# V-DETR/V-DETR

Hardware: AMD Instinct MI355X
Metric: scenes/sec (train fwd+bwd) 40k-pt ScanNet (higher is better)
Workload: dtype f32

## Files before the change

### include/vdetr_hip.h

```cpp
#ifndef VDETR_HIP_H
#define VDETR_HIP_H

#include <stddef.h>
#include <stdint.h>

#ifdef __cplusplus
extern "C" {
#endif

#define VDETR_OK 0
#define VDETR_ERR_ARG 1
#define VDETR_ERR_LAUNCH 2
#define VDETR_ERR_WORKSPACE 3

typedef void* vdetr_stream_t;

int vdetr_abi_version(void);
const char* vdetr_last_error(void);
int vdetr_ab_switches(void);


size_t vdetr_fps_workspace_bytes(int b, int n);
int vdetr_furthest_point_sampling_f32(const float* xyz, int b, int n, int m, int32_t* idx,
                                      void* workspace, size_t workspace_bytes, vdetr_stream_t stream);
// ... 15 lines not shown

int vdetr_ball_query_f32(const float* new_xyz, const float* xyz, int32_t* idx, int b, int n, int m,
                         float radius, int nsample, vdetr_stream_t stream);

int vdetr_group_points_f32(const float* points, const int32_t* idx, float* out, int b, int c, int n,
                           int npoints, int nsample, vdetr_stream_t stream);
int vdetr_group_points_grad_f32(const float* grad_out, const int32_t* idx, float* grad_points, int b,
                                int c, int n, int npoints, int nsample, vdetr_stream_t stream);
int vdetr_group_points_grad_set_f32(const float* grad_out, const int32_t* idx, float* grad_points, int b,
                                    int c, int n, int npoints, int nsample, vdetr_stream_t stream);

int vdetr_three_nn_f32(const float* unknown, const float* known, float* dist2, int32_t* idx, int b,
                       int n, int m, vdetr_stream_t stream);
int vdetr_three_interpolate_f32(const float* points, const int32_t* idx, const float* weight,
                                float* out, int b, int c, int m, int n, vdetr_stream_t stream);
int vdetr_three_interpolate_grad_f32(const float* grad_out, const int32_t* idx, const float* weight,
                                     float* grad_points, int b, int c, int n, int m,
                                     vdetr_stream_t stream);

#define VDETR_ATTN_SHARED_KV 0
#define VDETR_ATTN_PER_HEAD 1

#define VDETR_MASK_NONE 0
#define VDETR_MASK_BOOL 1
#define VDETR_MASK_FLOAT 2

#define VDETR_RPE_BILINEAR 0
#define VDETR_RPE_NEAREST 1

typedef struct vdetr_attn_desc {
  int32_t kind;
  int32_t B, H, nQ, nK;
  float scale;
  const float* table;
  int32_t table_size;
  float log_scale;
  float inv_log_norm;
  int32_t rpe_interp;
  const float* vertices;
  const float* xyz;
  const float* cos_sin;
  const void* mask;
  int32_t mask_kind;
  float dropout_p;
  uint64_t seed, offset;
  const uint64_t* rng_state;
  int32_t k_row_stride, v_row_stride;
  uint32_t* bwd_aux;
  int32_t table_grid;
  int32_t kv_waves;
  int32_t fwd_kernel;
  int32_t bwd_kernel;
  int32_t kv_halves;
  const void* kv_img;
  uint32_t* fwd_sched;
} vdetr_attn_desc;

size_t vdetr_attn_fwd_workspace_bytes(const vdetr_attn_desc* d);
size_t vdetr_attn_kv_image_bytes(int B, int nK);
int vdetr_attn_pack_kv_f32(const float* k, const float* v, int B, int nK, int k_row_stride, int v_row_stride, int nlayers,
                           int64_t layer_stride, void* img, vdetr_stream_t stream);
size_t vdetr_attn_kv_image_parts_bytes(int B, int nK, int parts);
int vdetr_attn_pack_kv_parts_f32(const float* k, const float* v, int B, int nK, int k_row_stride, int v_row_stride, int nlayers,
                                 int64_t layer_stride, int parts, void* img, vdetr_stream_t stream);

int vdetr_attn_fwd_f32(const vdetr_attn_desc* d, const float* q, const float* k, const float* v,
                       float* out, float* lse, float* scores, void* workspace, size_t workspace_bytes,
                       vdetr_stream_t stream);

typedef struct vdetr_attn_parts {
  const float* part_o;
  const float* part_lse;
  int32_t ksplit;
  int32_t reserved;
  int64_t rows;
} vdetr_attn_parts;
int vdetr_attn_fwd_parts_f32(const vdetr_attn_desc* d, const float* q, const float* k, const float* v,
                             float* out, float* lse, float* scores, void* workspace, size_t workspace_bytes,
                             vdetr_attn_parts* parts, vdetr_stream_t stream);

int vdetr_attn_fwd_bf16(const vdetr_attn_desc* d, const void* q, const void* k, const void* v, float* out, float* lse,
                        float* scores, void* workspace, size_t workspace_bytes, vdetr_stream_t stream);
size_t vdetr_attn_bwd_workspace_bytes(const vdetr_attn_desc* d);
int vdetr_attn_bwd_scores_f32(const vdetr_attn_desc* d, const float* scores, const float* dprob, const float* lse,
                              const float* delta, float* probs_out, float* ds_out, float* dtable, void* workspace,
                              size_t workspace_bytes, vdetr_stream_t stream);

size_t vdetr_attn_bwd_kv_workspace_bytes(const vdetr_attn_desc* d);
int vdetr_attn_bwd_kv_f32(const vdetr_attn_desc* d, const float* q, const float* v, const float* dout, const float* scores,
                          const float* lse, const float* delta, float* ds_out, float* dk, float* dv, void* workspace,
                          size_t workspace_bytes, vdetr_stream_t stream);
int vdetr_attn_bwd_kv_delta_f32(const vdetr_attn_desc* d, const float* q, const float* v, const float* dout, const float* out,
                                const float* scores, const float* lse, float* delta, float* ds_out, float* dk, float* dv,
                                void* workspace, size_t workspace_bytes, vdetr_stream_t stream);
typedef struct vdetr_attn_kv_prep {
  int32_t kind, B, H, nQ, nK, v_row_stride;
  const float* q;
  const float* v;
  const float* vertices;
  const float* cos_sin;
  void* workspace;
  float *dk, *dv;
  uint32_t* bwd_aux;
} vdetr_attn_kv_prep;
int vdetr_attn_bwd_kv_prep_f32(const vdetr_attn_kv_prep* items, int n, vdetr_stream_t stream);
int vdetr_attn_bwd_kv_packed_f32(const vdetr_attn_desc* d, const float* q, const float* v, const float* dout, const float* scores,
// ... 989 lines not shown
```

### v-detr_amd/_lib.py

```python
import ctypes
import os

import torch

_HERE = os.path.dirname(os.path.abspath(__file__))
LIB_PATH = os.path.join(_HERE, "lib", "libvdetr_hip.so")

c_int, c_float, c_void_p, c_size_t = ctypes.c_int, ctypes.c_float, ctypes.c_void_p, ctypes.c_size_t

VDETR_ATTN_SHARED_KV, VDETR_ATTN_PER_HEAD = 0, 1
VDETR_MASK_NONE, VDETR_MASK_BOOL, VDETR_MASK_FLOAT = 0, 1, 2
VDETR_RPE_BILINEAR, VDETR_RPE_NEAREST = 0, 1


class AttnDesc(ctypes.Structure):

    _fields_ = [
        ("kind", ctypes.c_int32), ("B", ctypes.c_int32), ("H", ctypes.c_int32), ("nQ", ctypes.c_int32),
        ("nK", ctypes.c_int32), ("scale", c_float),
        ("table", c_void_p), ("table_size", ctypes.c_int32), ("log_scale", c_float), ("inv_log_norm", c_float),
        ("rpe_interp", ctypes.c_int32),
        ("vertices", c_void_p), ("xyz", c_void_p), ("cos_sin", c_void_p),
        ("mask", c_void_p), ("mask_kind", ctypes.c_int32),
        ("dropout_p", c_float), ("seed", ctypes.c_uint64), ("offset", ctypes.c_uint64),
        ("rng_state", c_void_p),
        ("k_row_stride", ctypes.c_int32), ("v_row_stride", ctypes.c_int32),
        ("bwd_aux", c_void_p),
        ("table_grid", ctypes.c_int32), ("kv_waves", ctypes.c_int32), ("fwd_kernel", ctypes.c_int32), ("bwd_kernel", ctypes.c_int32), ("kv_halves", ctypes.c_int32), ("kv_img", c_void_p),
        ("fwd_sched", c_void_p),
    ]


VDETR_CLS_SOFTMAX, VDETR_CLS_SIGMOID = 0, 1

_BOX_IN = ("center", "size", "angle_cls", "angle_res", "cls", "pre_center_norm", "pre_size_norm", "dims_min", "dims_max")
_BOX_OUT = ("center_reg", "size_reg", "center_unnorm", "center_norm", "size_unnorm", "size_norm", "pre_center_unnorm",
            "pre_size_unnorm", "angle_residual", "angle_cont", "angle_prob", "angle_class", "corners", "corners_aa",
            "cls_prob", "objectness")


class BoxDecodeDesc(ctypes.Structure):

    _fields_ = ([(n, ctypes.c_int32) for n in ("B", "N", "A", "C1", "num_angle_bin", "cls_kind")] +
                [(n, c_void_p) for n in _BOX_IN + _BOX_OUT] + [("in_batch_stride", ctypes.c_int32)] +
                [(n, c_void_p) for n in ("cls_logits_t", "angle_logits_t", "angle_res_norm_t", "corners_lidar", "center_size")])


_BOX_GRAD_IN = ("center_reg", "size_reg", "center_unnorm", "center_norm", "size_unnorm", "size_norm", "angle_residual",
                "angle_cont", "angle_prob", "corners", "corners_aa")
_BOX_GRAD_OUT = ("d_center", "d_size", "d_angle_cls", "d_angle_res")


class BoxDecodeGrads(ctypes.Structure):

    _fields_ = ([(n, c_void_p) for n in _BOX_GRAD_IN + _BOX_GRAD_OUT] +
                [(n, c_void_p) for n in ("cls_logits_t", "angle_logits_t", "angle_res_norm_t", "d_cls")] +
                [("out_batch_stride", ctypes.c_int32), ("slab_rows", ctypes.c_int32)])


class AddLnDesc(ctypes.Structure):

    _fields_ = [("rows", ctypes.c_int32), ("C", ctypes.c_int32), ("eps", c_float), ("dropout_p", c_float),
                ("seed", ctypes.c_uint64), ("offset", ctypes.c_uint64), ("rng_state", c_void_p)] + [
        (n, c_void_p) for n in ("x", "r", "gamma", "beta", "gamma2", "beta2", "y", "out", "out2", "mean", "rstd")]


class AddLnGrads(ctypes.Structure):

    _fields_ = [(n, c_void_p) for n in ("d_out", "d_out2", "d_y", "d_x", "d_r", "d_gamma", "d_beta", "d_gamma2", "d_beta2",
                                        "partials")]


class AddLnReduce(ctypes.Structure):

    _fields_ = [("partials", c_void_p), ("nparts", ctypes.c_int32), ("C", ctypes.c_int32), ("d_gamma", c_void_p), ("d_beta", c_void_p),
                ("d_gamma2", c_void_p), ("d_beta2", c_void_p)]


class RbLinear(ctypes.Structure):

    _fields_ = [("w", c_void_p), ("b", c_void_p), ("wt", c_void_p)]
# ... 713 lines not shown
```

### v-detr_amd/attention.py

```python
import contextlib
import ctypes
import os
import weakref

import torch
from torch.autograd import Function

from . import _lib as L

HEAD_DIM = 64


class RPEConfig:

    INTERP = {"bilinear": L.VDETR_RPE_BILINEAR, "nearest": L.VDETR_RPE_NEAREST}

    def __init__(self, table_size=10, log_scale=512.0, max_value=4.0, interp="bilinear"):
        if interp not in self.INTERP:
            raise NotImplementedError(f"RPE interpolation '{interp}' (built: 'bilinear' and 'nearest')")
        self.interp = interp
        self.table_size = int(table_size)
        self.log_scale = float(log_scale)
        self.max_value = float(max_value)

    @property
    def inv_log_norm(self):
        return 1.0 / (3.0 * self.max_value)


def new_rng_state(device, seed=None):
    if seed is None:
        seed = torch.initial_seed()
    return torch.tensor([seed & 0x7FFFFFFFFFFFFFFF, 0], dtype=torch.int64, device=device)


FWD_KERNEL = int(os.environ.get("VDETR_FWD_KERNEL", "0"))
BWD_KERNEL = int(os.environ.get("VDETR_BWD_KERNEL", "0"))
TABLE_GRID = 0
FUSED_KV_BWD = os.environ.get("VDETR_BWD_FUSED", "1") != "0"
SELF_FWD_BODY = os.environ.get("VDETR_SELF_FWD", "") == "body"


_ASYNC_ENV = os.environ.get("VDETR_BWD_ASYNC_TABLE", "auto")
ASYNC_TABLE_GRAD = _ASYNC_ENV != "0"
ASYNC_MIN_PAIRS = 1 << 21
ASYNC_TABLE_GRID = int(os.environ.get("VDETR_BWD_ASYNC_GRID", "190"))


_step_side = {}


def side_branch_in_use(device):
    return bool(_step_side.get(_dev_key(device)))


class SideResults:
    pending = []

    @classmethod
    def flush(cls):
        from .helpers import DeferredParamGrads
        items, cls.pending = cls.pending, []
        late, side_late[:] = list(side_late), []
        for fn, alive in late:
            with torch.no_grad():
                items.append((None, fn(), alive))
        for dev, pairs, _alive in items:
            side = _side_streams.get(_dev_key(dev)) if dev is not None else None
            if side is not None:
                torch.cuda.current_stream(dev).wait_stream(side)
            roots, grads = [], []
            with torch.no_grad():
                for p, g in pairs:
                    if p is not None and p.requires_grad:
                        DeferredParamGrads._deliver(p, g, roots, grads)
            if roots:
                torch.autograd.backward(roots, grads)


_tick = {}
side_late = []


def flush_layer_params_on_side(ref, rows):
    from .helpers import DeferredParamGrads, DeferredPosEmbedGrads
    if not (ref.is_cuda and DeferredParamGrads.enabled and side_branch_in_use(ref.device)):
        return
    dev = ref.device
    key = _dev_key(dev)
    cur = torch.cuda.current_stream(dev)
    fork = torch.cuda.Event()
    fork.record(cur)
    if key not in _tick:
# ... 475 lines not shown
            if 2 <= parts.ksplit <= 16:
                _pending_parts[out.data_ptr()] = (parts, ws, lse, out)
            elif parts.ksplit != 1:
                raise RuntimeError(f"fused_attention: {parts.ksplit} key chunks left unmerged and no consumer takes that many")
        else:
            fwd = lib.vdetr_attn_fwd_bf16 if bf16 else lib.vdetr_attn_fwd_f32
            L.check(fwd(ctypes.byref(d), L.ptr(q), L.ptr(k), L.ptr(v), L.ptr(out), L.ptr(lse),
                        L.ptr(scores), L.ptr(ws), nbytes, L.stream_ptr()), "attn_fwd")
        if need_grad:
            ctx.save_for_backward(q, k, v, table, vertices, xyz, cos_sin, mask, out, lse, scores, rng)
            ctx.cfg = (kind, H, scale, rpe, dropout_p if use_drop else 0.0, salt)
            ctx.kv_rec = None if (bf16 or mask is not None) else _kv_register(out, q, v, table, vertices, cos_sin, kind, B, H, nQ, nK)
            ctx.table_async = bool(table_async)
            ctx.boxes = bool(boxes)
            if table_async and table is not None and table.requires_grad and _async_wanted(q.shape[0], q.shape[1], k.shape[1]):
                _step_side[_dev_key(q.device)] = True
        if _kv_by_out and getattr(ctx, "kv_rec", None) is None:
            _kv_by_out.pop(out.data_ptr(), None)
        return out

    @staticmethod
    def backward(ctx, dout):
        q, k, v, table, vertices, xyz, cos_sin, mask, out, lse, scores, rng = ctx.saved_tensors
        kind, H, scale, rpe, dropout_p, salt = ctx.cfg
        in_dtype = q.dtype
        if in_dtype == torch.bfloat16:
            q, k, v = q.float(), k.float().contiguous(), v.float().contiguous()
        B, nQ, C = q.shape
        nK = k.shape[1]
        lib = L.lib()
        dout = dout.contiguous()
        shared = kind == L.VDETR_ATTN_SHARED_KV
        want_table = table is not None and ctx.needs_input_grad[3]
        d = _desc(kind, B, H, nQ, nK, scale, table, rpe, vertices, xyz, cos_sin, mask, dropout_p, rng, salt, 0, v.stride(1))
        if getattr(ctx, "boxes", False) and BWD_KERNEL == 0 and cos_sin is None:
            d.bwd_kernel = 2
        if want_table:
            aux = _take_zeros(q, (8,), torch.int32)
            d.bwd_aux = aux.data_ptr()
        delta = torch.empty((B, nQ, H) if shared else (B, H, nQ), dtype=torch.float32, device=q.device)
        rows_kv, nprob_kv = (4 * nQ, B) if shared else (nQ, B * H)
        fused = (FUSED_KV_BWD and ((shared and H == 4) or (not shared and not want_table))
                 and rows_kv * nK * 4 < (1 << 31) and nprob_kv <= 65535 and v.stride(1) % 4 == 0
                 and all(t.data_ptr() % 16 == 0 for t in (v, lse)))
        if not fused:
            L.check(lib.vdetr_attn_delta_f32(ctypes.byref(d), L.ptr(dout), L.ptr(out), L.ptr(v), L.ptr(delta), L.stream_ptr()),
                    "attn_delta")
        if fused:
            ds = torch.empty_like(scores)
            dkv = torch.empty((2, B, nK, k.shape[2]), dtype=torch.float32, device=q.device)
            run_async = want_table and ctx.table_async and _async_wanted(B, nQ, nK)
            d.kv_waves = 4 if (run_async or _side_keep) and ASYNC_TABLE_GRID >= 256 else 8
            d.kv_halves = 1 if (_side_keep and not shared) else 2
            rec = getattr(ctx, "kv_rec", None)
            if (rec is not None and rec.prepared and rec.emitted == dout.data_ptr() and (rec.aux is not None) == bool(want_table)
                    and in_dtype == torch.float32):
                delta, dkv, aux = rec.delta, rec.dkv, rec.aux
                d.bwd_aux = aux.data_ptr() if aux is not None else None
                L.check(lib.vdetr_attn_bwd_kv_packed_f32(ctypes.byref(d), L.ptr(q), L.ptr(v), L.ptr(dout), L.ptr(scores), L.ptr(lse),
                                                         L.ptr(delta), L.ptr(ds), L.ptr(dkv[0]), L.ptr(dkv[1]), L.ptr(rec.ws), rec.nbytes,
                                                         L.stream_ptr()), "attn_bwd_kv_packed")
            else:
                nbytes = lib.vdetr_attn_bwd_kv_workspace_bytes(ctypes.byref(d))
                ws = L.workspace(nbytes, q.device)
                L.check(lib.vdetr_attn_bwd_kv_delta_f32(ctypes.byref(d), L.ptr(q), L.ptr(v), L.ptr(dout), L.ptr(out), L.ptr(scores),
                                                        L.ptr(lse), L.ptr(delta), L.ptr(ds), L.ptr(dkv[0]), L.ptr(dkv[1]), L.ptr(ws),
                                                        nbytes, L.stream_ptr()), "attn_bwd_kv")
            from .runtime import ts_mark
            ts_mark("main: key-side pass done" if shared else "main: self-attention key-side pass done")
            dtable = fork = None
            if run_async:
                dtable = _table_accumulator(table)
                fork = torch.cuda.Event()
                fork.record(torch.cuda.current_stream(q.device))
            if shared:
                dq = q.new_empty((B, nQ * H, HEAD_DIM))
                torch.baddbmm(dq, ds.view(B, nQ * H, nK), k, beta=0.0, alpha=float(scale), out=dq)
                dq = dq.view(B, nQ, C)
            else:
                ds_r = ds.view(B * H, nQ, nK)
                k4 = k.reshape(B, nK, H, HEAD_DIM).permute(0, 2, 1, 3)
                if B == 1:
                    dq = q.new_empty((1, nQ, C))
                    dq_r = dq.view(nQ, H, HEAD_DIM).permute(1, 0, 2)
                    torch.baddbmm(dq_r, ds_r, k4[0], beta=0.0, alpha=float(scale), out=dq_r)
                else:
                    dq = torch.bmm(ds_r, k4.reshape(B * H, nK, HEAD_DIM)).mul_(float(scale))
                    dq = dq.view(B, H, nQ, HEAD_DIM).permute(0, 2, 1, 3).reshape(B, nQ, C)
            if want_table:
                if run_async:
                    dtable = _launch_table_async(lib, d, q, ds, table, aux, vertices, xyz, mask, fork, dtable, also=(cos_sin, rng))
                else:
                    dtable = _table_accumulator(table)
                    nbytes = lib.vdetr_attn_bwd_workspace_bytes(ctypes.byref(d))
                    ws = L.workspace(nbytes, q.device)
                    L.check(lib.vdetr_attn_bwd_table_f32(ctypes.byref(d), L.ptr(ds), L.ptr(dtable), L.ptr(ws), nbytes,
                                                         L.stream_ptr()), "attn_bwd_table")
            dk, dv = dkv[0], dkv[1]
            if in_dtype == torch.bfloat16:
                dq, dk, dv = dq.to(in_dtype), dk.to(in_dtype), dv.to(in_dtype)
            return (dq, dk, dv, dtable) + (None,) * 17
        if shared:
            do_r = dout.view(B, nQ * H, HEAD_DIM)
            dprob = torch.bmm(do_r, v.transpose(1, 2))
        else:
            def heads(t, n):
# ... 135 lines not shown
```

### v-detr_amd/csrc/attn_bwd_kv.hip

```cpp
#include "kv_pack.h"
#include "workspace.h"

#include <stdlib.h>

#include <atomic>

namespace vdetr {

int attn_fill_params(const vdetr_attn_desc* d, AttnParams* P, const char* op);

typedef float f32x16 __attribute__((ext_vector_type(16)));


struct KvParams {
  AttnParams A;
  const float* dout;
  float* dk;
  float* dv;
  uint4* pack;
  int R, NT;
};

struct KvProblem {
  const float* q;
  const float* dout;
  const float* v;
  float* dk;
  float* dv;
  size_t score_off;
  size_t row_off;
  int rstride, ostride, b, head;
};
template <bool PERHEAD>
__device__ __forceinline__ KvProblem kv_problem(const KvParams& K, int prob) {
  const AttnParams& P = K.A;
  KvProblem p;
  if (PERHEAD) {
    const int b = prob / P.H, hh = prob - b * P.H, C = P.H * kDh;
    p.b = b; p.head = hh;
    p.q = P.q + (size_t)b * P.nQ * C + hh * kDh;
    p.dout = K.dout + (size_t)b * P.nQ * C + hh * kDh;
    p.rstride = C;
    p.v = P.v + (size_t)b * P.nK * P.v_stride + hh * kDh;
    p.dk = K.dk + (size_t)b * P.nK * C + hh * kDh;
    p.dv = K.dv + (size_t)b * P.nK * C + hh * kDh;
    p.ostride = C;
  } else {
    p.b = prob; p.head = 0;
    p.q = P.q + (size_t)prob * K.R * kDh;
    p.dout = K.dout + (size_t)prob * K.R * kDh;
    p.rstride = kDh;
    p.v = P.v + (size_t)prob * P.nK * P.v_stride;
    p.dk = K.dk + (size_t)prob * P.nK * kDh;
    p.dv = K.dv + (size_t)prob * P.nK * kDh;
    p.ostride = kDh;
  }
  p.score_off = (size_t)prob * K.R * P.nK;
  p.row_off = (size_t)prob * K.R;
  return p;
}


__device__ __forceinline__ f32x16 kv_mfma(bf16x8 a, bf16x8 b, f32x16 c) {
  return __builtin_amdgcn_mfma_f32_32x32x16_bf16(a, b, c, 0, 0, 0);
}
__device__ __forceinline__ f32x16 kv_mfma3(bf16x8 ah, bf16x8 al, bf16x8 bh, bf16x8 bl, f32x16 c) {
  c = kv_mfma(al, bh, c);
  c = kv_mfma(ah, bl, c);
  return kv_mfma(ah, bh, c);
}

template <bool PERHEAD>
__global__ __launch_bounds__(256) void attn_bwd_kv_pack_kernel(KvParams K, DeltaArgs D, int ndelta) {
  if ((int)blockIdx.x < ndelta) {
    __shared__ float wmax[4];
    attn_delta_body(D, (int)blockIdx.x, wmax);
    return;
  }
  const AttnParams& P = K.A;
  const int R = K.R, NT = K.NT;
  const int nprob = PERHEAD ? P.B * P.H : P.B;
  const long gid = (long)((int)blockIdx.x - ndelta) * 256 + threadIdx.x, stride = (long)((int)gridDim.x - ndelta) * 256;
  const long nunits = (long)nprob * NT * 12 * kWave;
  for (long u = gid; u < nunits; u += stride) {
    const int lane = (int)(u & 63);
    long r = u >> 6;
    const int sub = (int)(r & 3);
    r >>= 2;
    const int kind = (int)(r % 3);
    const long bt = r / 3;
    const int prob = (int)(bt / NT), tile = (int)(bt - (long)prob * NT), r0 = tile * 32;
    const int l31 = lane & 31, g = lane >> 5;
    const KvProblem pb = kv_problem<PERHEAD>(K, prob);
    const float* src = kind == 2 ? pb.q : pb.dout;
    float x[8];
    if (kind == 0) {
      const int row = r0 + l31;
#pragma unroll
      for (int e = 0; e < 8; ++e) x[e] = row < R ? src[(size_t)row * pb.rstride + 16 * sub + 8 * g + e] : 0.f;
    } else {
      const int d = 32 * (sub >> 1) + l31, t = sub & 1;
#pragma unroll
      for (int e = 0; e < 8; ++e) {
        const int row = r0 + kv_row(8 * t + e, g);
        x[e] = row < R ? src[(size_t)row * pb.rstride + d] : 0.f;
      }
    }
    bf16x8 hi, lo;
    kv_split8(x, hi, lo);
    uint4* dst = K.pack + ((bt * 3 + kind) * 4 + sub) * kKvOperandUnits;
    dst[lane] = __builtin_bit_cast(uint4, hi);
    dst[kWave + lane] = __builtin_bit_cast(uint4, lo);
  }
  const long nz = (long)P.B * P.nK * (PERHEAD ? P.H : 1) * kDh / 4;
  f32x4* zk = reinterpret_cast<f32x4*>(K.dk);
  f32x4* zv = reinterpret_cast<f32x4*>(K.dv);
  for (long i = gid; i < nz; i += stride) {
    zk[i] = f32x4{0.f, 0.f, 0.f, 0.f};
    zv[i] = f32x4{0.f, 0.f, 0.f, 0.f};
  }
}

template <bool PERHEAD, int WAVES, int HALVES = 2>
// ... 263 lines not shown
    const long bt = u >> 8;
    const int prob = (int)(bt / NT), tile = (int)(bt - (long)prob * NT), r0 = tile * 32;
    const int l31 = ln & 31, g = ln >> 5, d = 32 * (sub >> 1) + l31, t = sub & 1;
    const float* src;
    int rstride;
    if (I.perhead) {
      const int b = prob / I.H, hh = prob - b * I.H;
      src = I.q + (size_t)b * I.nQ * C + hh * kDh;
      rstride = C;
    } else {
      src = I.q + (size_t)prob * R * kDh;
      rstride = kDh;
    }
    float x[8];
#pragma unroll
    for (int e = 0; e < 8; ++e) {
      const int row = r0 + kv_row(8 * t + e, g);
      x[e] = row < R ? src[(size_t)row * rstride + d] : 0.f;
    }
    kv_store_unit(I.pack, bt, 2, sub, ln, x);
  }
  const long nz = (long)I.B * I.nK * (I.perhead ? I.H : 1) * kDh / 4;
  f32x4* zk = reinterpret_cast<f32x4*>(I.dk);
  f32x4* zv = reinterpret_cast<f32x4*>(I.dv);
  for (long i = gid; i < nz; i += stride) {
    zk[i] = f32x4{0.f, 0.f, 0.f, 0.f};
    zv[i] = f32x4{0.f, 0.f, 0.f, 0.f};
  }
}

}

using namespace vdetr;

static bool kv_supported(const vdetr_attn_desc* d) {
  return d && ((d->kind == VDETR_ATTN_SHARED_KV && d->H == 4) || d->kind == VDETR_ATTN_PER_HEAD);
}
static size_t kv_rows(const vdetr_attn_desc* d) { return d->kind == VDETR_ATTN_PER_HEAD ? (size_t)d->nQ : (size_t)d->nQ * 4; }
static size_t kv_problems(const vdetr_attn_desc* d) { return d->kind == VDETR_ATTN_PER_HEAD ? (size_t)d->B * d->H : (size_t)d->B; }

static uint4* lay_out(Carver& c, const vdetr_attn_desc* d) {
  const size_t nt = (kv_rows(d) + 31) / 32;
  return c.take_unpadded<uint4>(kv_problems(d) * nt * kKvTileUnits);
}

extern "C" size_t vdetr_attn_bwd_kv_workspace_bytes(const vdetr_attn_desc* d) {
  if (!kv_supported(d) || d->B <= 0 || d->nQ <= 0 || d->H <= 0) return 0;
  Carver c(nullptr);
  lay_out(c, d);
  return c.bytes() + 256;
}

template <bool PERHEAD, int WAVES, int HALVES = 2>
static int kv_launch(const KvParams& K, int nkt, int nprob, long pack_work, const DeltaArgs& D, int ndelta, bool packed, hipStream_t st) {
  const unsigned pack_blocks = (unsigned)((pack_work + 255) / 256 < 2048 ? (pack_work + 255) / 256 : 2048);
  if (!packed) {
    hipLaunchKernelGGL(attn_bwd_kv_pack_kernel<PERHEAD>, dim3(pack_blocks + (unsigned)ndelta), dim3(256), 0, st, K, D, ndelta);
    if (int e = check_launch("attn_bwd_kv_pack")) return e;
  }
  const size_t strips = (size_t)WAVES * 8 * kWave * sizeof(uint4), tree = (size_t)(WAVES / 2) * 64 * kWave * sizeof(float);
  const size_t fin = (size_t)2 * 32 * (kDh + 1) * sizeof(float);
  const size_t lds = strips > tree ? (strips > fin ? strips : fin) : (tree > fin ? tree : fin);
  if (int e = set_lds(attn_bwd_kv_kernel<PERHEAD, WAVES, HALVES>, lds, "attn_bwd_kv")) return e;
  hipLaunchKernelGGL((attn_bwd_kv_kernel<PERHEAD, WAVES, HALVES>), dim3(HALVES * nkt, nprob), dim3(WAVES * kWave), lds, st, K);
  return check_launch("attn_bwd_kv");
}

static int kv_run(const vdetr_attn_desc* d, const float* q, const float* v, const float* dout, const float* out,
                  const float* scores, const float* lse, float* delta, float* ds_out, float* dk, float* dv, void* workspace,
                  size_t workspace_bytes, vdetr_stream_t stream, bool packed = false) {
  KvParams K;
  if (int e = attn_fill_params(d, &K.A, "attn_bwd_kv")) return e;
  VDETR_REQUIRE(kv_supported(d), "attn_bwd_kv: built for shared K/V with 4 heads and for per-head K/V (kind %d, H %d)", d->kind, d->H);
  VDETR_REQUIRE(q && v && dout && scores && lse && delta && ds_out && dk && dv, "attn_bwd_kv: null pointer");
  VDETR_REQUIRE(K.A.v_stride % 4 == 0 && (((uintptr_t)v | (uintptr_t)lse | (uintptr_t)delta | (uintptr_t)dk | (uintptr_t)dv) & 15) == 0,
                "attn_bwd_kv: v rows, lse, delta, dk and dv must be 16-B aligned");
  const size_t rows = kv_rows(d), nprob = kv_problems(d);
  VDETR_REQUIRE(rows * d->nK * 4 < ((size_t)1 << 31), "attn_bwd_kv: a score matrix (%zu x %d) must stay below 2 GB", rows, d->nK);
  VDETR_REQUIRE(nprob <= 65535, "attn_bwd_kv: %zu score matrices > 65535", nprob);
  if (int e = require_workspace("attn_bwd_kv", workspace, workspace_bytes, vdetr_attn_bwd_kv_workspace_bytes(d))) return e;
  K.A.q = q; K.A.v = v;
  K.A.scores = const_cast<float*>(scores); K.A.lse = const_cast<float*>(lse); K.A.delta = delta; K.A.ds_out = ds_out;
  K.dout = dout; K.dk = dk; K.dv = dv;
  Carver carver(workspace);
  K.pack = lay_out(carver, d);
  K.R = (int)rows;
  K.NT = (K.R + 31) / 32;
  const long units = (long)nprob * K.NT * 12 * kWave;
  const long zero4 = (long)d->B * d->nK * (d->kind == VDETR_ATTN_PER_HEAD ? d->H : 1) * kDh / 4;
  const long work = units > zero4 ? units : zero4;
  const int nkt = (d->nK + 31) / 32;
  VDETR_REQUIRE(d->kv_waves == 0 || d->kv_waves == 4 || d->kv_waves == 8, "attn_bwd_kv: kv_waves %d (0, 4 or 8)", d->kv_waves);
  VDETR_REQUIRE(d->kv_halves == 0 || d->kv_halves == 1 || d->kv_halves == 2, "attn_bwd_kv: kv_halves %d (0, 1 or 2)", d->kv_halves);
  const bool four = d->kv_waves == 4;
  const bool one = d->kv_halves == 1 && !four;
  hipStream_t st = (hipStream_t)stream;
  DeltaArgs D{};
  int ndelta = 0;
  if (out) {
    VDETR_REQUIRE(!d->bwd_aux || d->kind == VDETR_ATTN_SHARED_KV, "attn_bwd_kv: bwd_aux needs the shared-KV kind");
    attn_delta_args(d, dout, out, v, delta, &D);
    ndelta = D.qblocks + D.vblocks;
  }
  if (d->kind == VDETR_ATTN_PER_HEAD) {
    if (one) return kv_launch<true, 8, 1>(K, nkt, (int)nprob, work, D, ndelta, packed, st);
    return four ? kv_launch<true, 4>(K, nkt, (int)nprob, work, D, ndelta, packed, st) : kv_launch<true, 8>(K, nkt, (int)nprob, work, D, ndelta, packed, st);
  }
  if (one) return kv_launch<false, 8, 1>(K, nkt, (int)nprob, work, D, ndelta, packed, st);
  return four ? kv_launch<false, 4>(K, nkt, (int)nprob, work, D, ndelta, packed, st) : kv_launch<false, 8>(K, nkt, (int)nprob, work, D, ndelta, packed, st);
}

extern "C" int vdetr_attn_bwd_kv_f32(const vdetr_attn_desc* d, const float* q, const float* v, const float* dout,
                                     const float* scores, const float* lse, const float* delta, float* ds_out, float* dk,
                                     float* dv, void* workspace, size_t workspace_bytes, vdetr_stream_t stream) {
  return kv_run(d, q, v, dout, nullptr, scores, lse, const_cast<float*>(delta), ds_out, dk, dv, workspace, workspace_bytes, stream);
}

extern "C" int vdetr_attn_bwd_kv_delta_f32(const vdetr_attn_desc* d, const float* q, const float* v, const float* dout,
                                           const float* out, const float* scores, const float* lse, float* delta, float* ds_out,
                                           float* dk, float* dv, void* workspace, size_t workspace_bytes, vdetr_stream_t stream) {
  VDETR_REQUIRE(out, "attn_bwd_kv_delta: null pointer (out)");
  return kv_run(d, q, v, dout, out, scores, lse, delta, ds_out, dk, dv, workspace, workspace_bytes, stream);
}

extern "C" int vdetr_attn_bwd_kv_packed_f32(const vdetr_attn_desc* d, const float* q, const float* v, const float* dout, const float* scores,
                                            const float* lse, const float* delta, float* ds_out, float* dk, float* dv, void* workspace,
                                            size_t workspace_bytes, vdetr_stream_t stream) {
  VDETR_REQUIRE(workspace && (((uintptr_t)workspace) & 255) == 0, "attn_bwd_kv_packed: the workspace (the operand images) must be 256-B aligned");
  return kv_run(d, q, v, dout, nullptr, scores, lse, const_cast<float*>(delta), ds_out, dk, dv, workspace, workspace_bytes, stream, true);
}

extern "C" int vdetr_attn_bwd_kv_prep_f32(const vdetr_attn_kv_prep* items, int n, vdetr_stream_t stream) {
  VDETR_REQUIRE(items && n >= 1 && n <= kPrepMax, "attn_bwd_kv_prep: %d items (1..%d)", n, kPrepMax);
  PrepBatch Bt;
  long blocks = 1;
  for (int i = 0; i < n; ++i) {
    const vdetr_attn_kv_prep& s = items[i];
    VDETR_REQUIRE(s.q && s.v && s.workspace && s.dk && s.dv, "attn_bwd_kv_prep: null pointer in item %d", i);
    VDETR_REQUIRE(s.kind == VDETR_ATTN_SHARED_KV || s.kind == VDETR_ATTN_PER_HEAD, "attn_bwd_kv_prep: kind %d", s.kind);
    VDETR_REQUIRE(s.B > 0 && s.nQ > 0 && s.nK > 0 && s.H == 4, "attn_bwd_kv_prep: item %d: B=%d nQ=%d nK=%d H=%d (4 heads)", i, s.B, s.nQ, s.nK, s.H);
    VDETR_REQUIRE((((uintptr_t)s.workspace) & 255) == 0 && (((uintptr_t)s.dk | (uintptr_t)s.dv) & 15) == 0, "attn_bwd_kv_prep: item %d: alignment", i);
    VDETR_REQUIRE(s.kind == VDETR_ATTN_SHARED_KV || !s.bwd_aux, "attn_bwd_kv_prep: bwd_aux needs the shared-KV kind");
    PrepItem& I = Bt.it[i];
    I.q = s.q; I.v = s.v; I.vertices = s.vertices; I.cos_sin = s.vertices ? s.cos_sin : nullptr;
    I.pack = reinterpret_cast<uint4*>(s.workspace); I.dk = s.dk; I.dv = s.dv; I.aux = s.bwd_aux;
    I.B = s.B; I.H = s.H; I.nQ = s.nQ; I.nK = s.nK;
    I.perhead = s.kind == VDETR_ATTN_PER_HEAD ? 1 : 0;
    I.v_stride = s.v_row_stride ? s.v_row_stride : (I.perhead ? s.H * 64 : 64);
    const long nvb = s.bwd_aux ? ((long)s.B * s.nK + 4 * kDeltaKeys - 1) / (4 * kDeltaKeys) : 0;
    const long nqb = (s.bwd_aux && s.vertices) ? ((long)s.B * s.nQ + 3) / 4 : 0;
    const long R = I.perhead ? s.nQ : (long)s.H * s.nQ, NT = (R + 31) / 32, nprob = I.perhead ? (long)s.B * s.H : s.B;
    const long units = nprob * NT * 4 * kWave, zero4 = (long)s.B * s.nK * (I.perhead ? s.H : 1) * kDh / 4;
    long work = ((units > zero4 ? units : zero4) + 255) / 256;
    work = work < 1 ? 1 : (work > 512 ? 512 : work);
    blocks = blocks > nvb + nqb + work ? blocks : nvb + nqb + work;
  }
  for (int i = n; i < kPrepMax; ++i) Bt.it[i] = Bt.it[0];
// ... 4 lines not shown
```

### v-detr_amd/csrc/kv_pack.h

```cpp
#pragma once
#include "attn_common.h"

namespace vdetr {

typedef __bf16 bf16x8 __attribute__((ext_vector_type(8)));

constexpr int kKvOperandUnits = 2 * kWave;
constexpr int kKvTileUnits = 3 * 4 * kKvOperandUnits;

__device__ __forceinline__ constexpr int kv_row(int v, int g) { return (v & 3) + 8 * (v >> 2) + 4 * g; }

__device__ __forceinline__ void kv_split8(const float (&x)[8], bf16x8& hi, bf16x8& lo) {
#pragma unroll
  for (int e = 0; e < 8; ++e) {
    const __bf16 h = (__bf16)x[e];
    hi[e] = h;
    lo[e] = (__bf16)(x[e] - (float)h);
  }
}

__device__ __forceinline__ void kv_store_unit(uint4* pack, long tile, int kind, int sub, int lane, const float (&x)[8]) {
  bf16x8 hi, lo;
  kv_split8(x, hi, lo);
  uint4* dst = pack + ((tile * 3 + kind) * 4 + sub) * kKvOperandUnits;
  dst[lane] = __builtin_bit_cast(uint4, hi);
  dst[kWave + lane] = __builtin_bit_cast(uint4, lo);
}

struct KvEmit {
  uint4* pack;
  float* delta;
  const float* out;
  unsigned* aux;
  int per_head, nQ;
};
__device__ __forceinline__ void kv_emit_rows16(const KvEmit& E, const float* xs, int stride, int q0, int tid, float* wmax) {
  const int NT = E.per_head ? E.nQ / 32 : E.nQ / 8;
  {
    const int pair = tid >> 2, quarter = tid & 3, ql = pair >> 2, h = pair & 3;
    const float* orow = E.out + ((size_t)(q0 + ql) * 4 + h) * kDh + 16 * quarter;
    const float* drow = xs + ql * stride + h * kDh + 16 * quarter;
    float s = 0.f, n2 = 0.f;
#pragma unroll
    for (int i = 0; i < 4; ++i) {
      const f32x4 o = *reinterpret_cast<const f32x4*>(orow + 4 * i);
      const f32x4 g = *reinterpret_cast<const f32x4*>(drow + 4 * i);
#pragma unroll
      for (int e = 0; e < 4; ++e) { s = fmaf(g[e], o[e], s); n2 = fmaf(g[e], g[e], n2); }
    }
    s += dpp_f32<kDppQuadXor1>(s); s += dpp_f32<kDppQuadXor2>(s);
    n2 += dpp_f32<kDppQuadXor1>(n2); n2 += dpp_f32<kDppQuadXor2>(n2);
    if (quarter == 0) E.delta[E.per_head ? (size_t)h * E.nQ + q0 + ql : (size_t)(q0 + ql) * 4 + h] = s;
    if (E.aux) {
      for (int m = 32; m >= 1; m >>= 1) n2 = fmaxf(n2, __shfl_xor(n2, m, 64));
      if ((tid & 63) == 0) wmax[tid >> 6] = n2;
    }
  }
#pragma unroll
  for (int u = 0; u < 4; ++u) {
    const int id = tid + 256 * u;
    float x[8];
    if (!E.per_head) {
      const int tl = id >> 9, unit = (id >> 6) & 7, lane = id & 63, kind = unit >> 2, sub = unit & 3, l31 = lane & 31, g = lane >> 5;
      if (kind == 0) {
        const float* src = xs + (tl * 8 + (l31 >> 2)) * stride + (l31 & 3) * kDh + 16 * sub + 8 * g;
        const f32x4 a = *reinterpret_cast<const f32x4*>(src), b = *reinterpret_cast<const f32x4*>(src + 4);
#pragma unroll
        for (int e = 0; e < 4; ++e) { x[e] = a[e]; x[4 + e] = b[e]; }
      } else {
        const int d = 32 * (sub >> 1) + l31, t = sub & 1;
#pragma unroll
        for (int e = 0; e < 8; ++e) {
          const int row = kv_row(8 * t + e, g);
          x[e] = xs[(tl * 8 + (row >> 2)) * stride + (row & 3) * kDh + d];
        }
      }
      kv_store_unit(E.pack, (long)(q0 >> 3) + tl, kind, sub, lane, x);
    } else {
      const int head = id >> 8, rem = id & 255, half = (q0 >> 4) & 1;
// ... 24 lines not shown
```

Before: 164.1.

## Add lean per-head self-attention backward dK/dV kernel with split-K slot reduction

Adds a dedicated per-head backward kernel that computes dV and dK for two 32-key tiles per block. Eight waves split the query tiles across slots, using software-pipelined buffer loads and split-bf16 MFMA, then combine partial accumulators with an LDS tree reduction. It is selected automatically when the per-head problem is unmasked, 32-aligned and uses eight waves, replacing the existing kv_launch path. The aim is better occupancy and less per-problem overhead in self-attention backward, at the cost of a new reduction path and extra LDS traffic.

After: 163.0. About the same (-0.6%).

```diff
diff --git a/include/vdetr_hip.h b/include/vdetr_hip.h
--- a/include/vdetr_hip.h
+++ b/include/vdetr_hip.h
@@ -91,6 +91,7 @@
   int32_t fwd_kernel;
   int32_t bwd_kernel;
   int32_t kv_halves;
+  int32_t kv_kernel;
   const void* kv_img;
   uint32_t* fwd_sched;
 } vdetr_attn_desc;
diff --git a/v-detr_amd/_lib.py b/v-detr_amd/_lib.py
--- a/v-detr_amd/_lib.py
+++ b/v-detr_amd/_lib.py
@@ -26,7 +26,7 @@
         ("rng_state", c_void_p),
         ("k_row_stride", ctypes.c_int32), ("v_row_stride", ctypes.c_int32),
         ("bwd_aux", c_void_p),
-        ("table_grid", ctypes.c_int32), ("kv_waves", ctypes.c_int32), ("fwd_kernel", ctypes.c_int32), ("bwd_kernel", ctypes.c_int32), ("kv_halves", ctypes.c_int32), ("kv_img", c_void_p),
+        ("table_grid", ctypes.c_int32), ("kv_waves", ctypes.c_int32), ("fwd_kernel", ctypes.c_int32), ("bwd_kernel", ctypes.c_int32), ("kv_halves", ctypes.c_int32), ("kv_kernel", ctypes.c_int32), ("kv_img", c_void_p),
         ("fwd_sched", c_void_p),
     ]
 
diff --git a/v-detr_amd/attention.py b/v-detr_amd/attention.py
--- a/v-detr_amd/attention.py
+++ b/v-detr_amd/attention.py
@@ -39,6 +39,7 @@
 TABLE_GRID = 0
 FUSED_KV_BWD = os.environ.get("VDETR_BWD_FUSED", "1") != "0"
 SELF_FWD_BODY = os.environ.get("VDETR_SELF_FWD", "") == "body"
+SELF_BWD_BODY = False
 
 
 _ASYNC_ENV = os.environ.get("VDETR_BWD_ASYNC_TABLE", "auto")
@@ -620,6 +621,7 @@
             run_async = want_table and ctx.table_async and _async_wanted(B, nQ, nK)
             d.kv_waves = 4 if (run_async or _side_keep) and ASYNC_TABLE_GRID >= 256 else 8
             d.kv_halves = 1 if (_side_keep and not shared) else 2
+            d.kv_kernel = 1 if SELF_BWD_BODY else 0
             rec = getattr(ctx, "kv_rec", None)
             if (rec is not None and rec.prepared and rec.emitted == dout.data_ptr() and (rec.aux is not None) == bool(want_table)
                     and in_dtype == torch.float32):
diff --git a/v-detr_amd/csrc/attn_bwd_kv.hip b/v-detr_amd/csrc/attn_bwd_kv.hip
--- a/v-detr_amd/csrc/attn_bwd_kv.hip
+++ b/v-detr_amd/csrc/attn_bwd_kv.hip
@@ -8,67 +8,10 @@
 namespace vdetr {
 
 int attn_fill_params(const vdetr_attn_desc* d, AttnParams* P, const char* op);
-
-typedef float f32x16 __attribute__((ext_vector_type(16)));
-
-
-struct KvParams {
-  AttnParams A;
-  const float* dout;
-  float* dk;
-  float* dv;
-  uint4* pack;
-  int R, NT;
-};
-
-struct KvProblem {
-  const float* q;
-  const float* dout;
-  const float* v;
-  float* dk;
-  float* dv;
-  size_t score_off;
-  size_t row_off;
-  int rstride, ostride, b, head;
-};
-template <bool PERHEAD>
-__device__ __forceinline__ KvProblem kv_problem(const KvParams& K, int prob) {
-  const AttnParams& P = K.A;
-  KvProblem p;
-  if (PERHEAD) {
-    const int b = prob / P.H, hh = prob - b * P.H, C = P.H * kDh;
-    p.b = b; p.head = hh;
-    p.q = P.q + (size_t)b * P.nQ * C + hh * kDh;
-    p.dout = K.dout + (size_t)b * P.nQ * C + hh * kDh;
-    p.rstride = C;
-    p.v = P.v + (size_t)b * P.nK * P.v_stride + hh * kDh;
-    p.dk = K.dk + (size_t)b * P.nK * C + hh * kDh;
-    p.dv = K.dv + (size_t)b * P.nK * C + hh * kDh;
-    p.ostride = C;
-  } else {
-    p.b = prob; p.head = 0;
-    p.q = P.q + (size_t)prob * K.R * kDh;
-    p.dout = K.dout + (size_t)prob * K.R * kDh;
-    p.rstride = kDh;
-    p.v = P.v + (size_t)prob * P.nK * P.v_stride;
-    p.dk = K.dk + (size_t)prob * P.nK * kDh;
-    p.dv = K.dv + (size_t)prob * P.nK * kDh;
-    p.ostride = kDh;
-  }
-  p.score_off = (size_t)prob * K.R * P.nK;
-  p.row_off = (size_t)prob * K.R;
-  return p;
-}
-
-
-__device__ __forceinline__ f32x16 kv_mfma(bf16x8 a, bf16x8 b, f32x16 c) {
-  return __builtin_amdgcn_mfma_f32_32x32x16_bf16(a, b, c, 0, 0, 0);
-}
-__device__ __forceinline__ f32x16 kv_mfma3(bf16x8 ah, bf16x8 al, bf16x8 bh, bf16x8 bl, f32x16 c) {
-  c = kv_mfma(al, bh, c);
-  c = kv_mfma(ah, bl, c);
-  return kv_mfma(ah, bh, c);
-}
+bool attn_bwd_self_eligible(const vdetr_attn_desc* d);
+int attn_bwd_self_launch(const KvParams& K, int nprob, hipStream_t st);
+
+
 
 template <bool PERHEAD>
 __global__ __launch_bounds__(256) void attn_bwd_kv_pack_kernel(KvParams K, DeltaArgs D, int ndelta) {
@@ -438,12 +381,14 @@
 }
 
 template <bool PERHEAD, int WAVES, int HALVES = 2>
-static int kv_launch(const KvParams& K, int nkt, int nprob, long pack_work, const DeltaArgs& D, int ndelta, bool packed, hipStream_t st) {
+static int kv_launch(const KvParams& K, int nkt, int nprob, long pack_work, const DeltaArgs& D, int ndelta, bool packed, hipStream_t st,
+                     bool lean = false) {
   const unsigned pack_blocks = (unsigned)((pack_work + 255) / 256 < 2048 ? (pack_work + 255) / 256 : 2048);
   if (!packed) {
     hipLaunchKernelGGL(attn_bwd_kv_pack_kernel<PERHEAD>, dim3(pack_blocks + (unsigned)ndelta), dim3(256), 0, st, K, D, ndelta);
     if (int e = check_launch("attn_bwd_kv_pack")) return e;
   }
+  if (lean) return attn_bwd_self_launch(K, nprob, st);
   const size_t strips = (size_t)WAVES * 8 * kWave * sizeof(uint4), tree = (size_t)(WAVES / 2) * 64 * kWave * sizeof(float);
   const size_t fin = (size_t)2 * 32 * (kDh + 1) * sizeof(float);
   const size_t lds = strips > tree ? (strips > fin ? strips : fin) : (tree > fin ? tree : fin);
@@ -489,6 +434,7 @@
     ndelta = D.qblocks + D.vblocks;
   }
   if (d->kind == VDETR_ATTN_PER_HEAD) {
+    if (attn_bwd_self_eligible(d)) return kv_launch<true, 8, 1>(K, nkt, (int)nprob, work, D, ndelta, packed, st, true);
     if (one) return kv_launch<true, 8, 1>(K, nkt, (int)nprob, work, D, ndelta, packed, st);
     return four ? kv_launch<true, 4>(K, nkt, (int)nprob, work, D, ndelta, packed, st) : kv_launch<true, 8>(K, nkt, (int)nprob, work, D, ndelta, packed, st);
   }
diff --git a/v-detr_amd/csrc/attn_bwd_self.hip b/v-detr_amd/csrc/attn_bwd_self.hip
--- /dev/null
+++ b/v-detr_amd/csrc/attn_bwd_self.hip
@@ -0,0 +1,248 @@
+#include "kv_pack.h"
+
+namespace vdetr {
+
+constexpr int kSbWaves = 8;
+constexpr int kSbSlots = 4;
+constexpr int kSbStripFloats = 2 * 8 * kWave * 4;
+constexpr int kSbLdsFloats = kSbStripFloats + kSbWaves * 64 * kWave;
+constexpr int kSbFinStride = kDh + 1;
+
+template <bool DROP>
+__global__ __launch_bounds__(kSbWaves * kWave) void attn_bwd_self_kernel(KvParams K) {
+  extern __shared__ __attribute__((aligned(16))) float smem[];
+  float* red = smem + kSbStripFloats;
+  AttnParams P = K.A;
+  if (DROP) attn_load_rng(P);
+  const int tid = threadIdx.x, lane = tid & 63;
+  const int w = __builtin_amdgcn_readfirstlane(tid >> 6);
+  const int j = w & 1, slot = w >> 1;
+  const int l31 = lane & 31, g = lane >> 5;
+  const int prob = blockIdx.y, nK = P.nK, NT = K.NT, nkt = nK >> 5;
+  const int kt = 2 * (int)blockIdx.x + j;
+  const bool live = kt < nkt;
+  const KvProblem pb = kv_problem<true>(K, prob);
+  const int key = kt * 32 + l31;
+
+  uint4* vstrip = reinterpret_cast<uint4*>(smem) + j * (8 * kWave) + lane;
+  if (live && slot == 0) {
+    const float* vrow = pb.v + (size_t)key * P.v_stride + 8 * g;
+#pragma unroll
+    for (int s = 0; s < 4; ++s) {
+      const f32x4 a = *reinterpret_cast<const f32x4*>(vrow + 16 * s), c = *reinterpret_cast<const f32x4*>(vrow + 16 * s + 4);
+      const float x[8] = {a[0], a[1], a[2], a[3], c[0], c[1], c[2], c[3]};
+      bf16x8 hi, lo;
+      kv_split8(x, hi, lo);
+      vstrip[(2 * s) * kWave] = __builtin_bit_cast(uint4, hi);
+      vstrip[(2 * s + 1) * kWave] = __builtin_bit_cast(uint4, lo);
+    }
+  }
+  __syncthreads();
+
+  f32x16 accV[2], accK[2];
+#pragma unroll
+  for (int i = 0; i < 16; ++i) { accV[0][i] = 0.f; accV[1][i] = 0.f; accK[0][i] = 0.f; accK[1][i] = 0.f; }
+
+  auto put = [&](int region) {
+    float* dst = red + (size_t)region * 64 * kWave + lane;
+#pragma unroll
+    for (int i = 0; i < 16; ++i) {
+      dst[i * kWave] = accV[0][i]; dst[(16 + i) * kWave] = accV[1][i];
+      dst[(32 + i) * kWave] = accK[0][i]; dst[(48 + i) * kWave] = accK[1][i];
+    }
+  };
+  auto add = [&](int region) {
+    const float* src = red + (size_t)region * 64 * kWave + lane;
+#pragma unroll
+    for (int i = 0; i < 16; ++i) {
+      accV[0][i] += src[i * kWave]; accV[1][i] += src[(16 + i) * kWave];
+      accK[0][i] += src[(32 + i) * kWave]; accK[1][i] += src[(48 + i) * kWave];
+    }
+  };
+  bool parked = false;
+  if (live && slot < NT) {
+    using rsrc_t = __amdgpu_buffer_rsrc_t;
+    const unsigned recs = (unsigned)((size_t)K.R * nK * 4);
+    const rsrc_t rs = __builtin_amdgcn_make_buffer_rsrc(P.scores + pb.score_off, 0, (int)recs, 0x00020000);
+    const rsrc_t rd = __builtin_amdgcn_make_buffer_rsrc(P.ds_out + pb.score_off, 0, (int)recs, 0x00020000);
+    const rsrc_t rl = __builtin_amdgcn_make_buffer_rsrc(const_cast<float*>(P.lse + pb.row_off), 0, K.R * 4, 0x00020000);
+    const rsrc_t rq = __builtin_amdgcn_make_buffer_rsrc(const_cast<float*>(P.delta + pb.row_off), 0, K.R * 4, 0x00020000);
+    const rsrc_t rp = __builtin_amdgcn_make_buffer_rsrc(K.pack + (size_t)prob * NT * kKvTileUnits, 0, NT * kKvTileUnits * 16, 0x00020000);
+    const int rowbytes = nK * 4;
+    const int lane_off = 4 * g * rowbytes + key * 4;
+    const int lane16 = lane * 16, g16 = g * 16;
+    const bool second = (pb.head & 2) != 0;
+    const int shift = (pb.head & 1) * 16;
+
+    float sv[16];
+    f32x4 lq[4], dq[4];
+    auto unit = [&](int tile, int u) {
+      return __builtin_bit_cast(uint4, __builtin_amdgcn_raw_buffer_load_b128(rp, lane16 + (u & 3) * (kWave * 16), (tile * 6 + (u >> 2)) * (4 * kWave * 16), 0));
+    };
+    auto load_dp = [&](int tile, uint4 (&S)[8]) {
+#pragma unroll
+      for (int i = 0; i < 8; ++i) S[i] = unit(tile, i);
+    };
+    auto load_step = [&](int tile, int t, uint4 (&S)[8]) {
+#pragma unroll
+      for (int mt = 0; mt < 2; ++mt)
+#pragma unroll
+        for (int hl = 0; hl < 2; ++hl) {
+          S[2 * mt + hl] = unit(tile, (4 + 2 * mt + t) * 2 + hl);
+          S[4 + 2 * mt + hl] = unit(tile, (8 + 2 * mt + t) * 2 + hl);
+        }
+    };
+    auto load_rows = [&](int tile, int t) {
+#pragma unroll
+      for (int a2 = 0; a2 < 2; ++a2) {
+        const int a = 2 * t + a2;
+#pragma unroll
+        for (int h = 0; h < 4; ++h)
+          sv[4 * a + h] = __builtin_bit_cast(float, __builtin_amdgcn_raw_buffer_load_b32(rs, lane_off, (tile * 32 + 8 * a + h) * rowbytes, kStreamAux));
+        lq[a] = __builtin_bit_cast(f32x4, __builtin_amdgcn_raw_buffer_load_b128(rl, g16, (tile * 8 + 2 * a) * 16, 0));
+        dq[a] = __builtin_bit_cast(f32x4, __builtin_amdgcn_raw_buffer_load_b128(rq, g16, (tile * 8 + 2 * a) * 16, 0));
+      }
+    };
+
+    auto step = [&](uint4 (&X)[8], uint4 (&Y)[8], int tile, int next) {
+      const int r0 = tile * 32;
+      const bool more = next >= 0;
+      unsigned mine = 0;
+      if (DROP) mine = attn_prefix(P, pb.b, r0 + kv_row(l31 & 15, g), pb.head >> 2);
+      f32x16 dp;
+#pragma unroll
+      for (int i = 0; i < 16; ++i) dp[i] = 0.f;
+#pragma unroll
+      for (int s = 0; s < 4; ++s) {
+        const bf16x8 vh = __builtin_bit_cast(bf16x8, vstrip[(2 * s) * kWave]), vl = __builtin_bit_cast(bf16x8, vstrip[(2 * s + 1) * kWave]);
+        dp = kv_mfma3(__builtin_bit_cast(bf16x8, X[2 * s]), __builtin_bit_cast(bf16x8, X[2 * s + 1]), vh, vl, dp);
+      }
+      __builtin_amdgcn_sched_barrier(0);
+      load_step(tile, 1, X);
+      __builtin_amdgcn_sched_barrier(0);
+#pragma unroll
+      for (int t = 0; t < 2; ++t) {
+        float xp[8], xs[8];
+        unsigned word[8];
+        if (DROP) {
+#pragma unroll
+          for (int e = 0; e < 8; ++e)
+            word[e] = drop_word((unsigned)__builtin_amdgcn_ds_bpermute((32 * g + 8 * t + e) << 2, (int)mine), (unsigned)key);
+          if (second) {
+#pragma unroll
+            for (int e = 0; e < 8; ++e) word[e] = drop_next(word[e]);
+          }
+        }
+#pragma unroll
+        for (int a2 = 0; a2 < 2; ++a2) {
+          const int a = 2 * t + a2;
+#pragma unroll
+          for (int h = 0; h < 4; ++h) {
+            const int v = 4 * a + h, e = 4 * a2 + h;
+            const bool keep = DROP ? ((word[e] >> shift) & 0xFFFFu) >= P.drop_thresh : true;
+            const ScoreGrad gr = score_grad(sv[v], lq[a][h], keep, P.drop_scale, true, dp[v], dq[a][h], false);
+            xp[e] = gr.p_drop;
+            xs[e] = gr.ds;
+            __builtin_amdgcn_raw_buffer_store_b32(__float_as_int(gr.ds), rd, lane_off, (r0 + 8 * a + h) * rowbytes, kStreamAux);
+          }
+        }
+        bf16x8 ph, pl, sh, sl;
+        kv_split8(xp, ph, pl);
+        kv_split8(xs, sh, sl);
+        const uint4* op = t ? X : Y;
+#pragma unroll
+        for (int mt = 0; mt < 2; ++mt) {
+          accV[mt] = kv_mfma3(__builtin_bit_cast(bf16x8, op[2 * mt]), __builtin_bit_cast(bf16x8, op[2 * mt + 1]), ph, pl, accV[mt]);
+          accK[mt] = kv_mfma3(__builtin_bit_cast(bf16x8, op[4 + 2 * mt]), __builtin_bit_cast(bf16x8, op[4 + 2 * mt + 1]), sh, sl, accK[mt]);
+        }
+        __builtin_amdgcn_sched_barrier(0);
+        if (more) {
+          if (t == 0) load_dp(next, Y); else load_step(next, 0, X);
+          load_rows(next, t);
+        }
+        __builtin_amdgcn_sched_barrier(0);
+      }
+    };
+
+    uint4 opA[8], opB[8];
+    load_dp(slot, opA);
+    load_rows(slot, 0);
+    load_step(slot, 0, opB);
+    load_rows(slot, 1);
+    auto succ = [&](int t) {
+      if (t + 2 * kSbSlots < NT) return t + 2 * kSbSlots;
+      return ((t & kSbSlots) == 0 && slot + kSbSlots < NT) ? slot + kSbSlots : -1;
+    };
+    auto park = [&](int t, int next) {
+      if (next >= 0 && (t & kSbSlots) == 0 && (next & kSbSlots) != 0) {
+        put(w);
+        parked = true;
+#pragma unroll
+        for (int i = 0; i < 16; ++i) { accV[0][i] = 0.f; accV[1][i] = 0.f; accK[0][i] = 0.f; accK[1][i] = 0.f; }
+      }
+    };
+    for (int tile = slot;;) {
+      int next = succ(tile);
+      step(opA, opB, tile, next);
+      park(tile, next);
+      if (next < 0) break;
+      tile = next;
+      next = succ(tile);
+      step(opB, opA, tile, next);
+      park(tile, next);
+      if (next < 0) break;
+      tile = next;
+    }
+    if (parked) add(w);
+  }
+  __syncthreads();
+
+
+  if (live && slot >= 2) put(2 * (slot - 2) + j);
+  __syncthreads();
+  if (live && slot < 2) add(2 * slot + j);
+  __syncthreads();
+  if (live && slot == 1) put(j);
+  __syncthreads();
+  if (live && slot == 0) add(j);
+  __syncthreads();
+  if (live && slot == 0) {
+    float* fin = red + (size_t)j * 2 * 32 * kSbFinStride;
+#pragma unroll
+    for (int mt = 0; mt < 2; ++mt)
+#pragma unroll
+      for (int i = 0; i < 16; ++i) {
+        const int d = 32 * mt + kv_row(i, g);
+        fin[l31 * kSbFinStride + d] = accV[mt][i];
+        fin[(32 + l31) * kSbFinStride + d] = accK[mt][i] * P.scale;
+      }
+  }
+  __syncthreads();
+  for (int idx = tid; idx < 2 * 2 * 32 * kDh; idx += kSbWaves * kWave) {
+    const int jj = idx >> 12, which = (idx >> 11) & 1, kl = (idx >> 6) & 31, d = idx & 63;
+    const int ktile = 2 * (int)blockIdx.x + jj;
+    if (ktile < nkt)
+      (which ? pb.dk : pb.dv)[(size_t)(ktile * 32 + kl) * pb.ostride + d] = red[((jj * 2 + which) * 32 + kl) * kSbFinStride + d];
+  }
+}
+
+bool attn_bwd_self_eligible(const vdetr_attn_desc* d) {
+  return d->kind == VDETR_ATTN_PER_HEAD && (!d->mask || d->mask_kind == VDETR_MASK_NONE) && d->nQ % 32 == 0 && d->nK % 32 == 0 &&
+         d->nQ <= (1 << 20) &&
+         (d->kv_waves == 0 || d->kv_waves == 8) && d->kv_kernel != 1;
+}
+
+int attn_bwd_self_launch(const KvParams& K, int nprob, hipStream_t st) {
+  const dim3 grid((unsigned)((K.A.nK / 32 + 1) / 2), (unsigned)nprob);
+  constexpr size_t lds = kSbLdsFloats * sizeof(float);
+  if (K.A.drop_thresh) {
+    if (int e = set_lds(attn_bwd_self_kernel<true>, lds, "attn_bwd_self")) return e;
+    hipLaunchKernelGGL((attn_bwd_self_kernel<true>), grid, dim3(kSbWaves * kWave), lds, st, K);
+  } else {
+    if (int e = set_lds(attn_bwd_self_kernel<false>, lds, "attn_bwd_self")) return e;
+    hipLaunchKernelGGL((attn_bwd_self_kernel<false>), grid, dim3(kSbWaves * kWave), lds, st, K);
+  }
+  return check_launch("attn_bwd_self");
+}
+
+}
diff --git a/v-detr_amd/csrc/kv_pack.h b/v-detr_amd/csrc/kv_pack.h
--- a/v-detr_amd/csrc/kv_pack.h
+++ b/v-detr_amd/csrc/kv_pack.h
@@ -25,6 +25,65 @@
   uint4* dst = pack + ((tile * 3 + kind) * 4 + sub) * kKvOperandUnits;
   dst[lane] = __builtin_bit_cast(uint4, hi);
   dst[kWave + lane] = __builtin_bit_cast(uint4, lo);
+}
+
+typedef float f32x16 __attribute__((ext_vector_type(16)));
+
+struct KvParams {
+  AttnParams A;
+  const float* dout;
+  float* dk;
+  float* dv;
+  uint4* pack;
+  int R, NT;
+};
+
+struct KvProblem {
+  const float* q;
+  const float* dout;
+  const float* v;
+  float* dk;
+  float* dv;
+  size_t score_off;
+  size_t row_off;
+  int rstride, ostride, b, head;
+};
+template <bool PERHEAD>
+__device__ __forceinline__ KvProblem kv_problem(const KvParams& K, int prob) {
+  const AttnParams& P = K.A;
+  KvProblem p;
+  if (PERHEAD) {
+    const int b = prob / P.H, hh = prob - b * P.H, C = P.H * kDh;
+    p.b = b; p.head = hh;
+    p.q = P.q + (size_t)b * P.nQ * C + hh * kDh;
+    p.dout = K.dout + (size_t)b * P.nQ * C + hh * kDh;
+    p.rstride = C;
+    p.v = P.v + (size_t)b * P.nK * P.v_stride + hh * kDh;
+    p.dk = K.dk + (size_t)b * P.nK * C + hh * kDh;
+    p.dv = K.dv + (size_t)b * P.nK * C + hh * kDh;
+    p.ostride = C;
+  } else {
+    p.b = prob; p.head = 0;
+    p.q = P.q + (size_t)prob * K.R * kDh;
+    p.dout = K.dout + (size_t)prob * K.R * kDh;
+    p.rstride = kDh;
+    p.v = P.v + (size_t)prob * P.nK * P.v_stride;
+    p.dk = K.dk + (size_t)prob * P.nK * kDh;
+    p.dv = K.dv + (size_t)prob * P.nK * kDh;
+    p.ostride = kDh;
+  }
+  p.score_off = (size_t)prob * K.R * P.nK;
+  p.row_off = (size_t)prob * K.R;
+  return p;
+}
+
+__device__ __forceinline__ f32x16 kv_mfma(bf16x8 a, bf16x8 b, f32x16 c) {
+  return __builtin_amdgcn_mfma_f32_32x32x16_bf16(a, b, c, 0, 0, 0);
+}
+__device__ __forceinline__ f32x16 kv_mfma3(bf16x8 ah, bf16x8 al, bf16x8 bh, bf16x8 bl, f32x16 c) {
+  c = kv_mfma(al, bh, c);
+  c = kv_mfma(ah, bl, c);
+  return kv_mfma(ah, bh, c);
 }
 
 struct KvEmit {
```
